# SilverlightningY/dmmt-jpeg-encoder

Hardware: AMD Instinct MI355X
Metric: Mpixel/s encoded (4K PPM, q=90) (higher is better)
Workload: dtype f32; 1 GPU; 3840x2160 synthetic RGB u8, 4:4:4, IJG quality 90, 1 frame(s) per step per GPU, pixels in HBM -> JPEG files in HBM, inputs rotating over 12 distinct slots (285 MiB: streamed from HBM); width=3840, height=2160, subsampling=P444, quality=90, parallelism=independent frames x1, lanes=4, input_slots=12

## Files before the change

dmmt-jpeg-encoder_amd/csrc/entropy.hip:

```cpp
#include <hip/hip_runtime.h>
#include <stdint.h>

#include "device_common.hpp"
#include "jpeg_common.hpp"
#include "kernels.hpp"
#include "slot_copy.hpp"

namespace dmmt {

#ifdef DMMT_PHASE_TRACE
static __device__ unsigned long long g_trace[64];
#endif

static_assert(kChunkBlocks == 256 || kChunkBlocks == 512, "one thread per block, one workgroup per chunk");
constexpr int kEmitThreads = kChunkBlocks;
constexpr int kEmitWaves = kEmitThreads / 64;
#ifndef DMMT_EMIT_OCC
#define DMMT_EMIT_OCC 7
#endif
constexpr int kEmitOcc = kChunkBlocks == 256 ? DMMT_EMIT_OCC : 3;

constexpr int kEmitWords = 4 * kChunkBlocks;
constexpr int kStuffPass = 4096;
#ifndef DMMT_EMIT_BRANCHFREE
#define DMMT_EMIT_BRANCHFREE 1
#endif
#ifndef DMMT_TAIL_DMA
#define DMMT_TAIL_DMA 1
#endif
#ifndef DMMT_TAIL_NSEG1
#define DMMT_TAIL_NSEG1 1
#endif
#ifndef DMMT_EMIT_PRIO_ALWAYS
#define DMMT_EMIT_PRIO_ALWAYS 0
#endif
#ifndef DMMT_EMIT_PRIO
#define DMMT_EMIT_PRIO 1
#endif

struct ChunkSpan {
    long long el0;
    int nb;
    int seg;
    bool seg_first, seg_last;
};

__device__ __forceinline__ ChunkSpan chunk_span(const Geom& g, int c) {
    ChunkSpan r;
    r.seg = min(c / g.cps, g.nseg - 1);
    const int j = c - r.seg * g.cps;
    const long long sb = (long long)r.seg * g.seg_blocks;
    const long long se = min(sb + g.seg_blocks, g.bpf);
    r.el0 = sb + (long long)j * kChunkBlocks;
    r.nb = (int)min((long long)kChunkBlocks, se - r.el0);
    r.seg_first = j == 0;
    r.seg_last = r.el0 + r.nb == se;
    return r;
}

__device__ __forceinline__ bool joined_tail(const Geom& g, int c) {
    return c == g.nch - 1 && g.more_after && g.restart_interval == 0;
}

__device__ __forceinline__ int mod_small(int x, int d, uint32_t inv16) {
    return x - (int)__umul24((uint32_t)d, __umul24((uint32_t)x, inv16) >> 16);
}

struct BlockCoef {
    uint32_t w[32];
};

__device__ __forceinline__ void load_block(const int16_t* __restrict__ p, BlockCoef& b) {
    const uint4* q = reinterpret_cast<const uint4*>(p);
#pragma unroll
    for (int i = 0; i < 8; ++i) {
        const uint4 v = q[i];
        b.w[4 * i] = v.x;
        b.w[4 * i + 1] = v.y;
        b.w[4 * i + 2] = v.z;
        b.w[4 * i + 3] = v.w;
    }
}

__device__ __forceinline__ int coef_at(const BlockCoef& b, int k) {
    return (k & 1) ? ((int)b.w[k >> 1] >> 16) : (int)(int16_t)(b.w[k >> 1] & 0xFFFFu);
}

__device__ __forceinline__ void zigzag_in_registers(BlockCoef& b) {
    uint32_t z[32];
#pragma unroll
    for (int j = 0; j < 32; ++j) {
        const int i0 = coef_pos(2 * j), i1 = coef_pos(2 * j + 1);
        const uint32_t lo = (b.w[i0 >> 1] >> (16 * (i0 & 1))) & 0xFFFFu;
        const uint32_t hi = (b.w[i1 >> 1] >> (16 * (i1 & 1))) & 0xFFFFu;
        z[j] = lo | (hi << 16);
    }
#pragma unroll
    for (int j = 0; j < 32; ++j) b.w[j] = z[j];
}

template <typename Sink>
__device__ __forceinline__ void walk_block(const BlockCoef& b, int dcd, const uint2* __restrict__ dctab,
                                           const uint2* __restrict__ actab, Sink& sink, int kmax = 63) {
    {
        const int cat = category_of(dcd);
        const uint2 e = dctab[cat];
        sink(e.x | extra_bits(dcd, cat), (int)e.y);
    }
    const uint2 z = actab[0xF0];
    uint32_t m_run = 0xF0u, m_low = 0xFFFFu, m_zrl = 255u;
    asm volatile("" : "+s"(m_run), "+s"(m_low), "+s"(m_zrl));
    int l16 = 16;
#pragma unroll
    for (int k0 = 0; k0 < 64; k0 += 4) {
        if (k0 != 0 && k0 > kmax) break;
#pragma unroll
        for (int k = k0 ? k0 : 1; k < k0 + 4; ++k) {
            const uint32_t w = b.w[k >> 1];
            if ((k & 1) ? w > m_low : (w << 16) != 0u) {
                const int v = coef_at(b, k);
                const int r16 = 16 * k - l16;
                if (k >= 17 && __builtin_amdgcn_ballot_w64((uint32_t)r16 > m_zrl) != 0) {
                    int r = r16 >> 8;
                    asm volatile("" : "+v"(r));
#pragma unroll 1
                    for (; r > 0; --r) sink(z.x, (int)z.y);
                }
                const int cat = category_fast(v);
                const uint2 e = actab[(r16 & (int)m_run) | cat];
                sink(e.x | extra_bits(v, cat), (int)e.y);
                l16 = 16 * k + 16;
            }
        }
    }
    if (l16 < 16 * 64 || kmax < 63) {
        const uint2 e = actab[0];
        sink(e.x, (int)e.y);
    }
}

struct CountSink {
    uint32_t n = 0;
    __device__ __forceinline__ void operator()(uint32_t, int len) { n += (uint32_t)len; }
};

struct WindowSink {
    uint32_t* img;
    int lo, n;
    unsigned long long acc;
    int nacc;
    int w;
    bool first;
    __device__ __forceinline__ void put(uint32_t word, bool shared) {
        const int i = w - lo;
        if ((unsigned)i < (unsigned)n) {
            if (shared)
                atomicOr(&img[i], word);
            else
                img[i] = word;
        }
    }
    __device__ __forceinline__ void operator()(uint32_t val, int len) {
        acc = (acc << len) | val;
        nacc += len;
        if (nacc >= 32) {
            nacc -= 32;
            put((uint32_t)(acc >> nacc), first);
            first = false;
            ++w;
        }
    }
    __device__ __forceinline__ void finish() {
        if (nacc > 0) put((uint32_t)(acc << (32 - nacc)), true);
    }
};


struct SlotSink {
    uint32_t* slot;
    unsigned long long acc;
    int nacc;
    int wi;
#if DMMT_EMIT_BRANCHFREE
    __device__ __forceinline__ void operator()(uint32_t val, int len) {
        acc = (acc << len) | val;
        nacc += len;
        const int full = nacc >> 5;
        nacc &= 31;
        slot[min(wi, kSlotWords - 1) * kEmitThreads] = (uint32_t)(acc >> nacc);
        wi += full;
    }
#else
    __device__ __forceinline__ void operator()(uint32_t val, int len) {
        acc = (acc << len) | val;
        nacc += len;
        if (nacc >= 32) {
            nacc -= 32;
            slot[min(wi, kSlotWords - 1) * kEmitThreads] = (uint32_t)(acc >> nacc);
            ++wi;
        }
    }
#endif
    __device__ __forceinline__ uint32_t finish() {
        if (nacc > 0 && wi < kSlotWords) slot[wi * kEmitThreads] = (uint32_t)(acc << (32 - nacc));
        return (uint32_t)wi * 32u + (uint32_t)nacc;
    }
};


__device__ __forceinline__ uint32_t bits16_at(uint32_t a, uint32_t b, int p) {
    const unsigned long long x = ((unsigned long long)a << 32) | b;
    return (uint32_t)(x >> (48 - (p & 31))) & 0xFFFFu;
}

struct NoMark {
    template <typename I>
    __device__ void operator()(I) const {}
};
template <typename Mark = NoMark>
__device__ __forceinline__ void fused_offsets(const uint32_t* __restrict__ cbits, const uint32_t* __restrict__ cff,
                              const unsigned long long* __restrict__ cff8, uint8_t* sFF8,
                              const uint32_t* __restrict__ cedge, const Geom& g, unsigned long long* __restrict__ bit0,
                              unsigned long long* __restrict__ outo, unsigned long long* __restrict__ total,
                              unsigned long long* sWaveV, int* sWaveF, Mark mark = Mark());
static_assert(kArriveWords == kArriveFrameWords, "the host sizes the counters");

__global__ __launch_bounds__(kEmitThreads, kEmitOcc) void k_emit(const int16_t* coef, const int16_t* __restrict__ dcdiff,
                                              const uint8_t* __restrict__ lastnz,
                                              const uint32_t* __restrict__ code_tab, Geom g,
                                              uint32_t* __restrict__ stage, uint32_t* __restrict__ chunk_bits,
                                              uint32_t* __restrict__ chunk_ff, uint32_t* __restrict__ chunk_edge,
                                              uint32_t* __restrict__ ac_hist, uint32_t* __restrict__ dc_hist,
                                              int fuse, uint32_t* __restrict__ arrive,
                                              unsigned long long* __restrict__ chunk_bit0,
                                              unsigned long long* __restrict__ chunk_out,
                                              unsigned long long* __restrict__ total_out,
                                              unsigned long long* __restrict__ chunk_ff8, int prio) {
    __shared__ uint2 sTab[2 * 256 + 2 * 16];
    __shared__ uint32_t sW[kEmitWords + 2];
    __shared__ __attribute__((aligned(16))) uint32_t sSlot[kSlotWords * kEmitThreads];
    __shared__ uint32_t sWave[kEmitWaves];
    __shared__ uint32_t sFF[8];
    __shared__ uint32_t sEdge[3];
    __shared__ uint32_t sBin[65];
    __shared__ unsigned long long sOffV[kEmitWaves + 1];
    __shared__ int sOffF[kEmitWaves];
    __shared__ uint32_t sLast;
    using OrderT = std::conditional_t<(kEmitThreads > 256), uint16_t, uint8_t>;
    uint32_t* const sBits = sW;
    OrderT* const sOrder = reinterpret_cast<OrderT*>(sW + kEmitThreads);
    uint8_t* const sKey = reinterpret_cast<uint8_t*>(sW + kEmitThreads + kEmitThreads * (int)sizeof(OrderT) / 4);
    DMMT_TRACE_START;
    const int tid = threadIdx.x, lane = lane_id(), wave = tid >> 6;
    const int frame = blockIdx.y;
    const unsigned chunk = blockIdx.x;
    const ChunkSpan span = chunk_span(g, (int)chunk);
    const long long el0 = span.el0;
    const int nb = span.nb;
    const long long e = (long long)frame * g.bpf + el0 + tid;
    const size_t cid = (size_t)frame * g.nch + chunk;
    const int r0 = (int)((uint32_t)el0 % (uint32_t)g.bpm);
    const uint32_t inv16 = (65536u + (uint32_t)g.bpm - 1u) / (uint32_t)g.bpm;
    const bool valid = tid < nb;
    const uint32_t* ct = code_tab + (size_t)frame * 1024;
    const int tt = tid & 255;
    const uint32_t tac0 = ct[256 + tt], tac1 = ct[768 + tt];
    const uint32_t tdc = ct[((tt & 31) < 16 ? 0 : 512 - 16) + (tt & 31)];
    const uint32_t lz = lastnz[valid ? e : (long long)frame * g.bpf + el0];
    if (tid < 256) {
        const int c = tid & 15;
        sTab[tid] = make_uint2((tac0 & 0xFFFFu) << c, (tac0 >> 16) + c);
        sTab[256 + tid] = make_uint2((tac1 & 0xFFFFu) << c, (tac1 >> 16) + c);
    }
    if (tid < 32) sTab[512 + tid] = make_uint2((tdc & 0xFFFFu) << (tid & 15), (tdc >> 16) + (tid & 15));
    if (chunk == 0) {
        for (int i = tid; i < kHistReps * 512; i += kEmitThreads) ac_hist[(size_t)frame * kHistReps * 512 + i] = 0u;
        for (int i = tid; i < kHistReps * 32; i += kEmitThreads) dc_hist[(size_t)frame * kHistReps * 32 + i] = 0u;
    }
    if (tid < 8) sFF[tid] = 0u;
    if (tid < 3) sEdge[tid] = 0u;
    if (tid < 65) sBin[tid] = 0u;
    const int key = valid ? (int)lz : 64;
    __syncthreads();
    const uint32_t rank = atomicAdd(&sBin[key], 1u);
    __syncthreads();
    if (tid < 64) {
        const uint32_t c = sBin[tid];
        const uint32_t inc = wave_incl_scan_full_u32(c);
        sBin[tid] = inc - c;
    }
    __syncthreads();
    const int mine = valid ? (int)(sBin[key] + rank) : tid;
    if (valid) {
        sOrder[mine] = (OrderT)tid;
        sKey[mine] = (uint8_t)key;
    }
    __syncthreads();
    DMMT_TRACE(0);
    uint32_t wbits = 0;
    bool slot_over = false;
    {
#if DMMT_EMIT_PRIO
        if (prio) {
            if (wave == 3) __builtin_amdgcn_s_setprio(3);
            else if (wave == 2) __builtin_amdgcn_s_setprio(2);
            else if (wave == 1) __builtin_amdgcn_s_setprio(1);
        }
#endif
        if (valid) {
            const int p = sOrder[tid];
            const long long ep = (long long)frame * g.bpf + el0 + p;
            BlockCoef b;
            load_block(coef + ep * 64, b);
            zigzag_in_registers(b);
            const int dp = dcdiff[ep];
            DMMT_TRACE(4);
            const int kp = mod_small(r0 + p, g.bpm, inv16);
            const bool lum = kp < g.n_luma;
            const int kmax = __builtin_amdgcn_readfirstlane((int)sKey[min(64 * wave + 63, nb - 1)]);
            SlotSink ss{sSlot + tid, 0ull, 0, 0};
            walk_block(b, dp, sTab + 512 + (lum ? 0 : 16), sTab + (lum ? 0 : 256), ss, kmax);
            wbits = ss.finish();
            slot_over = wbits > (uint32_t)kSlotWords * 32u;
            sBits[p] = wbits;
            DMMT_TRACE(5);
        }
    }
#if DMMT_EMIT_PRIO
    if (prio) __builtin_amdgcn_s_setprio(0);
#endif
    const bool over = __syncthreads_or(slot_over) != 0;
    const uint32_t bits = valid ? sBits[tid] : 0u;
    const int k = valid ? mod_small(r0 + tid, g.bpm, inv16) : 0;
    const bool lum_t = k < g.n_luma;
    const uint32_t incl = wave_incl_scan_full_u32(bits);
    if (lane == 63) sWave[wave] = incl;
    __syncthreads();
    uint32_t start = incl - bits;
    uint32_t total = 0;
#pragma unroll
    for (int q = 0; q < kEmitWaves; ++q) {
        start += q < wave ? sWave[q] : 0u;
        total += sWave[q];
    }
    DMMT_TRACE(1);

    uint32_t* slot = stage + cid * (size_t)kChunkWordsCap;
    const int nw = (int)((total + 31) >> 5);
    const int we1 = total >= 16 ? (int)((total - 16) >> 5) : 0;
    uint32_t ff[8] = {0, 0, 0, 0, 0, 0, 0, 0};
    for (int w0 = 0; w0 < nw; w0 += kEmitWords) {
        const int wn = min(kEmitWords, nw - w0);
        if (!over) {
            SlotWords sw;
            read_slot<kEmitThreads>(sSlot, mine, bits, sw);
            if (tid == 0 && w0 + wn >= nw) sW[wn] = 0u;
            copy_owned(sw, start, bits, sW, w0, wn);
            __syncthreads();
            copy_head(sw, start, bits, sW, w0, wn);
        } else {
            for (int i = tid; i <= wn; i += kEmitThreads) sW[i] = 0u;
            __syncthreads();
        }
        if (over && bits && start < (uint32_t)(w0 + wn + 1) * 32u && start + bits > (uint32_t)w0 * 32u) {
            {
                BlockCoef b;
                load_block(coef + e * 64, b);
                zigzag_in_registers(b);
                WindowSink ws{sW, w0, wn + 1, 0ull, (int)(start & 31), (int)(start >> 5), true};
                walk_block(b, dcdiff[e], sTab + 512 + (lum_t ? 0 : 16), sTab + (lum_t ? 0 : 256), ws);
                ws.finish();
            }
        }
        __syncthreads();
        for (int i = tid; i < wn; i += kEmitThreads) {
            const uint32_t a = sW[i], c = sW[i + 1];
            slot[w0 + i] = a;
            const int wi = w0 + i;
            if (wi == 0) sEdge[0] = a;
            if (wi == we1) {
                sEdge[1] = a;
                sEdge[2] = c;
            }
            const unsigned long long x = ((unsigned long long)a << 32) | c;
            unsigned long long z = x & (x << 1);
            z &= z << 2;
            z &= z << 4;
            const uint32_t m = (uint32_t)(z >> 32);
            if (m) {
#pragma unroll
                for (int r = 0; r < 8; ++r) ff[r] += __popc(m & (0x80808080u >> r));
            }
        }
        __syncthreads();
    }
    DMMT_TRACE(2);
#pragma unroll
    for (int r = 0; r < 4; ++r) {
        const uint32_t v = wave_sum_full_u32(ff[2 * r] | (ff[2 * r + 1] << 16));
        if (lane == 0 && v) {
            atomicAdd(&sFF[2 * r], v & 0xFFFFu);
            atomicAdd(&sFF[2 * r + 1], v >> 16);
        }
    }
    __syncthreads();
    if (tid == 0) {
        const uint32_t first16 = sEdge[0] >> 16;
        uint32_t last16;
        if (total >= 16)
            last16 = bits16_at(sEdge[1], sEdge[2], (int)(total - 16));
        else
            last16 = total ? sEdge[0] >> (32 - total) : 0u;
        unsigned long long f8 = 0;
#pragma unroll
        for (int r = 0; r < 8; ++r) {
            __hip_atomic_store(chunk_ff + cid * 8 + r, sFF[r], __ATOMIC_RELAXED, __HIP_MEMORY_SCOPE_AGENT);
            f8 |= (unsigned long long)min(sFF[r], 255u) << (8 * r);
        }
        __hip_atomic_store(chunk_ff8 + cid, f8, __ATOMIC_RELAXED, __HIP_MEMORY_SCOPE_AGENT);
        __hip_atomic_store(chunk_bits + cid, total, __ATOMIC_RELAXED, __HIP_MEMORY_SCOPE_AGENT);
        __hip_atomic_store(chunk_edge + cid, (first16 << 16) | last16, __ATOMIC_RELAXED, __HIP_MEMORY_SCOPE_AGENT);
    }
    if (fuse) {
        if (tid == 0) sLast = arrive_last(arrive + (size_t)frame * kArriveWords, chunk, (unsigned)g.nch);
        __syncthreads();
        DMMT_TRACE(6);
        if (sLast) {
            arrive_acquire();
            const size_t fb = (size_t)frame * g.nch;
#ifdef DMMT_PHASE_TRACE
            auto mark = [&](auto i) { DMMT_TRACE(decltype(i)::value); };
#else
            NoMark mark;
#endif
            fused_offsets(chunk_bits + fb, chunk_ff + fb * 8, chunk_ff8 + fb, reinterpret_cast<uint8_t*>(sSlot),
                          chunk_edge + fb, g, chunk_bit0 + fb, chunk_out + fb, total_out + frame, sOffV, sOffF, mark);
        }
    }
    DMMT_TRACE(3);
    DMMT_TRACE_FLUSH(0, 0);
}

__device__ __forceinline__ uint32_t boundary_byte(int m1, uint32_t last16, bool has_next, uint32_t n_next,
                                                  uint32_t first16_next) {
    uint32_t v = last16 & ((1u << m1) - 1u);
    int m2 = 8 - m1;
    if (has_next) {
        const int t = (int)min((uint32_t)m2, n_next);
        v = (v << t) | (t ? first16_next >> (16 - t) : 0u);
        m2 -= t;
    }
    return ((v << m2) | ((1u << m2) - 1u)) & 0xFFu;
}

__device__ __forceinline__ unsigned long long chunk_out_bytes(const uint32_t* __restrict__ cff,
                                                              const uint32_t* __restrict__ cbits,
                                                              const uint32_t* __restrict__ cedge, const Geom& g,
                                                              int c, unsigned long long b0) {
    const ChunkSpan sp = chunk_span(g, c);
    const uint32_t n = cbits[c];
    const unsigned long long e = b0 + n;
    unsigned long long out = ((e + 7) >> 3) - ((b0 + 7) >> 3);
    out += cff[(size_t)c * 8 + ((8 - (b0 & 7)) & 7)];
    if ((e & 7) && (e & ~7ull) >= b0) {
        const bool jt = joined_tail(g, c);
        const bool has_next = !sp.seg_last || jt;
        const uint32_t nn = jt ? (uint32_t)g.next_bits : (has_next ? cbits[c + 1] : 0u);
        const uint32_t fn = jt ? g.next16 : (has_next ? cedge[c + 1] >> 16 : 0u);
        const uint32_t byte = boundary_byte((int)(e & 7), cedge[c] & 0xFFFFu, has_next, nn, fn);
        out += byte == 0xFFu ? 1u : 0u;
    }
    if (sp.seg_last && (c != g.nch - 1 || (g.more_after && g.restart_interval > 0))) out += 2;
    return out;
}

template <int NW>
__device__ __forceinline__ unsigned long long block_scan_nw(unsigned long long v, unsigned long long* sWave,
                                                            unsigned long long* tot) {
    const int lane = lane_id(), wave = threadIdx.x >> 6;
    const unsigned long long incl = wave_incl_scan_full_u64(v);
    if (lane == 63) sWave[wave] = incl;
    __syncthreads();
    unsigned long long pre = incl - v, all = 0;
    for (int q = 0; q < NW; ++q) {
        if (q < wave) pre += sWave[q];
        all += sWave[q];
    }
    __syncthreads();
    *tot = all;
    return pre;
}

__device__ __forceinline__ void seg_combine(bool& f, unsigned long long& v, bool f2, unsigned long long v2) {
    v = f2 ? v2 : v + v2;
    f = f || f2;
}

template <int NW>
__device__ __forceinline__ unsigned long long block_segscan_nw(bool f, unsigned long long v,
                                                               unsigned long long* sWaveV, int* sWaveF,
                                                               bool* flag_out = nullptr) {
    const int lane = lane_id(), wave = threadIdx.x >> 6;
    bool fi = f;
    unsigned long long vi = v;
    auto step = [&](unsigned long long pv, int pf) {
        bool ff = pf != 0;
        seg_combine(ff, pv, fi, vi);
        fi = ff;
        vi = pv;
    };
    step(dpp_u64<0x111, 0xF, 0xF, true>(vi), __builtin_amdgcn_update_dpp(0, (int)fi, 0x111, 0xF, 0xF, true));
    step(dpp_u64<0x112, 0xF, 0xF, true>(vi), __builtin_amdgcn_update_dpp(0, (int)fi, 0x112, 0xF, 0xF, true));
    step(dpp_u64<0x114, 0xF, 0xF, true>(vi), __builtin_amdgcn_update_dpp(0, (int)fi, 0x114, 0xF, 0xF, true));
    step(dpp_u64<0x118, 0xF, 0xF, true>(vi), __builtin_amdgcn_update_dpp(0, (int)fi, 0x118, 0xF, 0xF, true));
    step(dpp_u64<0x142, 0xA, 0xF, false>(vi), __builtin_amdgcn_update_dpp(0, (int)fi, 0x142, 0xA, 0xF, false));
    step(dpp_u64<0x143, 0xC, 0xF, false>(vi), __builtin_amdgcn_update_dpp(0, (int)fi, 0x143, 0xC, 0xF, false));
    if (lane == 63) {
        sWaveV[wave] = vi;
        sWaveF[wave] = fi;
    }
    const unsigned long long ve = dpp_u64<0x138, 0xF, 0xF, true>(vi);
    const int fe = __builtin_amdgcn_update_dpp(0, (int)fi, 0x138, 0xF, 0xF, true);
    __syncthreads();
    bool cf = false;
    unsigned long long cv = 0;
    for (int q = 0; q < wave; ++q) seg_combine(cf, cv, sWaveF[q] != 0, sWaveV[q]);
    bool rf = cf;
    unsigned long long rv = cv;
    seg_combine(rf, rv, fe != 0, ve);
    __syncthreads();
    if (flag_out) *flag_out = rf;
    return rv;
}

__device__ __forceinline__ unsigned long long block_scan_1024(unsigned long long v, unsigned long long* sWave,
                                                              unsigned long long* tot) {
    return block_scan_nw<16>(v, sWave, tot);
}
__device__ __forceinline__ unsigned long long block_segscan_1024(bool f, unsigned long long v,
                                                                 unsigned long long* sWaveV, int* sWaveF) {
    return block_segscan_nw<16>(f, v, sWaveV, sWaveF);
}

static_assert(kFusedRoundChunks % kEmitThreads == 0, "whole chunks per thread of the fused offsets");
static_assert(kFusedRoundChunks % (2 * kEmitThreads) == 0 && kFusedRoundChunks * 8 <= kSlotWords * kEmitThreads * 4,
              "a round's packed 0xFF counts: whole 16-byte pieces per thread, inside k_emit's slot area");
static_assert((unsigned long long)kFusedOffsetsMaxChunks * kChunkBlocks * kMaxBlockBits < (1ull << 32),
              "a fused frame's bit offsets fit 32 bits");
template <typename Mark>
__device__ __forceinline__ void fused_offsets(const uint32_t* __restrict__ cbits, const uint32_t* __restrict__ cff,
                              const unsigned long long* __restrict__ cff8, uint8_t* sFF8,
                              const uint32_t* __restrict__ cedge, const Geom& g, unsigned long long* __restrict__ bit0,
                              unsigned long long* __restrict__ outo, unsigned long long* __restrict__ total,
                              unsigned long long* sWaveV, int* sWaveF, Mark mark) {
    constexpr int KP = kFusedRoundChunks / kEmitThreads, NT = kEmitThreads;
    const int tid = threadIdx.x;
    const int nch = g.nch;
    uint32_t carry_run = 0, carry_out = 0;
    for (int r0 = 0; r0 < nch; r0 += kFusedRoundChunks) {
        const int rn = min(kFusedRoundChunks, nch - r0);
        const int per = (rn + NT - 1) / NT;
        const int c0 = r0 + min(tid * per, rn), c1 = r0 + min(tid * per + per, rn);
#if DMMT_TAIL_DMA
        {
            const int npairs = (rn + 1) >> 1;
#pragma unroll
            for (int i = 0; i < kFusedRoundChunks / 2 / NT; ++i) {
                const int pc = min(i * NT + tid, npairs - 1);
                __builtin_amdgcn_global_load_lds((const void*)(cff8 + r0 + 2 * pc),
                                                 (void*)(sFF8 + 16 * (i * NT + (tid & ~63))), 16, 0, 16);
            }
        }
#endif
        uint32_t nbits[KP], edge[KP];
#pragma unroll
        for (int i = 0; i < KP; ++i) {
            const int c = min(c0 + i, nch - 1);
            nbits[i] = ld_agent(cbits + c);
            edge[i] = ld_agent(cedge + c);
        }
        const int cl = min(c1, nch - 1);
        const uint32_t nlast = ld_agent(cbits + cl), elast = ld_agent(cedge + cl);
        uint32_t firstm = 0, seglm = 0;
#pragma unroll
        for (int i = 0; i < KP; ++i) nbits[i] = c0 + i < c1 ? nbits[i] : 0u;
        if (DMMT_TAIL_NSEG1 && g.nseg == 1) {
            firstm = c0 == 0 && c0 < c1 ? 1u : 0u;
            seglm = c1 == nch && c0 < c1 ? 1u << (c1 - 1 - c0) : 0u;
        } else {
#pragma unroll
            for (int i = 0; i < KP; ++i) {
                const int c = c0 + i;
                if (c < c1) {
                    const ChunkSpan sp = chunk_span(g, c);
                    firstm |= (uint32_t)sp.seg_first << i;
                    seglm |= (uint32_t)sp.seg_last << i;
                }
            }
        }
        bool f = false;
        unsigned long long v = 0;
#pragma unroll
        for (int i = 0; i < KP; ++i)
            if (c0 + i < c1) seg_combine(f, v, (firstm >> i) & 1u, nbits[i] + (c0 + i == 0 ? (uint32_t)g.bit_phase : 0u));
        bool fx;
        const uint32_t ex = (uint32_t)block_segscan_nw<kEmitWaves>(f, v, sWaveV, sWaveF, &fx);
        mark(std::integral_constant<int, 7>{});
        uint32_t run = fx ? ex : carry_run + ex;
        uint32_t b0[KP];
#pragma unroll
        for (int i = 0; i < KP; ++i) {
            b0[i] = 0;
            if (c0 + i < c1) {
                if ((firstm >> i) & 1u) run = c0 + i == 0 ? (uint32_t)g.bit_phase : 0u;
                b0[i] = run;
                run += nbits[i];
            }
        }
        if (c0 < c1 && c1 == r0 + rn) sWaveV[kEmitWaves] = run;
        uint32_t ob[KP];
#if DMMT_TAIL_DMA
#pragma unroll
        for (int i = 0; i < KP; ++i) {
            const int cc = min(c0 + i, nch - 1);
            const uint32_t slot = (8u - (b0[i] & 7u)) & 7u;
            ob[i] = sFF8[8 * (cc - r0) + slot];
            if (ob[i] == 255u) ob[i] = ld_agent(cff + (size_t)cc * 8 + slot);
        }
#else
#pragma unroll
        for (int i = 0; i < KP; ++i)
            ob[i] = ld_agent(cff + (size_t)min(c0 + i, nch - 1) * 8 + ((8 - (b0[i] & 7)) & 7));
#endif
        uint32_t mine = 0;
#pragma unroll
        for (int i = 0; i < KP; ++i) {
            const int c = c0 + i;
            if (c >= c1) {
                ob[i] = 0;
                continue;
            }
            const uint32_t e = b0[i] + nbits[i];
            uint32_t o = ((e + 7) >> 3) - ((b0[i] + 7) >> 3) + ob[i];
            if ((e & 7) && (e & ~7u) >= b0[i]) {
                const bool segl = (seglm >> i) & 1u;
                const bool jt = segl && joined_tail(g, c);
                const bool hasn = !segl || jt;
                const uint32_t nn = jt ? (uint32_t)g.next_bits : i + 1 < KP && c + 1 < c1 ? nbits[min(i + 1, KP - 1)] : nlast;
                const uint32_t en = jt ? g.next16 << 16 : i + 1 < KP && c + 1 < c1 ? edge[min(i + 1, KP - 1)] : elast;
                const uint32_t byte = boundary_byte((int)(e & 7), edge[i] & 0xFFFFu, hasn, nn, en >> 16);
                o += byte == 0xFFu ? 1u : 0u;
            }
            if (((seglm >> i) & 1u) && (c != nch - 1 || (g.more_after && g.restart_interval > 0))) o += 2;
            ob[i] = o;
            mine += o;
        }
        mark(std::integral_constant<int, 8>{});
        unsigned long long tot = 0;
        uint32_t orun = carry_out + (uint32_t)block_scan_nw<kEmitWaves>(mine, sWaveV, &tot);
        mark(std::integral_constant<int, 9>{});
#pragma unroll
        for (int i = 0; i < KP; ++i) {
            const int c = c0 + i;
            if (c >= c1) continue;
            bit0[c] = b0[i];
            outo[c] = orun;
            orun += ob[i];
        }
        carry_out += (uint32_t)tot;
        carry_run = (uint32_t)sWaveV[kEmitWaves];
        __syncthreads();
        mark(std::integral_constant<int, 10>{});
    }
    if (tid == 0) *total = carry_out;
}

__global__ __launch_bounds__(1024) void k_offsets(const uint32_t* __restrict__ chunk_bits,
                                                  const uint32_t* __restrict__ chunk_ff,
                                                  const uint32_t* __restrict__ chunk_edge, Geom g,
                                                  unsigned long long* __restrict__ chunk_bit0,
                                                  unsigned long long* __restrict__ chunk_out,
                                                  unsigned long long* __restrict__ total_out) {
    __shared__ unsigned long long sWave[16];
    __shared__ int sWaveF[16];
    const int tid = threadIdx.x;
    const int frame = blockIdx.x;
    const int nch = g.nch;
    const uint32_t* cbits = chunk_bits + (size_t)frame * nch;
    const uint32_t* cff = chunk_ff + (size_t)frame * nch * 8;
    const uint32_t* cedge = chunk_edge + (size_t)frame * nch;
    unsigned long long* bit0 = chunk_bit0 + (size_t)frame * nch;
    unsigned long long* outo = chunk_out + (size_t)frame * nch;
    const int per = (nch + 1023) / 1024;
    const int c0 = min(tid * per, nch), c1 = min(c0 + per, nch);

    constexpr int KP = 2;
    if (per <= KP) {
        uint32_t nbits[KP], ffr[KP][8], edge[KP], nnext[KP], enext[KP];
        bool first[KP], segl[KP], hasn[KP];
#pragma unroll
        for (int i = 0; i < KP; ++i) {
            const int c = c0 + i;
            nbits[i] = edge[i] = nnext[i] = enext[i] = 0u;
            first[i] = segl[i] = hasn[i] = false;
#pragma unroll
            for (int r = 0; r < 8; ++r) ffr[i][r] = 0u;
            if (c < c1) {
                const ChunkSpan sp = chunk_span(g, c);
                first[i] = sp.seg_first;
                segl[i] = sp.seg_last;
                hasn[i] = !sp.seg_last;
                nbits[i] = cbits[c];
// ... 194 lines not shown
        if (lane == 63) sWave[wave] = incl;
        __syncthreads();
        uint32_t pre = incl - cnt;
        for (int q = 0; q < wave; ++q) pre += sWave[q];
        const uint32_t ffs = sWave[0] + sWave[1] + sWave[2] + sWave[3];
        if (nvalid) {
            const uint32_t dst = delta + (uint32_t)tid * 16u + pre;
            uint32_t a = dst;
#pragma unroll
            for (int i = 0; i < 4; ++i) {
                const uint32_t w = x[i], f = ffm[i];
                sOut[a + 4 * i] = (uint8_t)(w >> 24);
                sOut[a + (uint32_t)__popc(f & 0x80000000u) + 4 * i + 1] = (uint8_t)(w >> 16);
                sOut[a + (uint32_t)__popc(f & 0x80800000u) + 4 * i + 2] = (uint8_t)(w >> 8);
                sOut[a + (uint32_t)__popc(f & 0x80808000u) + 4 * i + 3] = (uint8_t)w;
                a += (uint32_t)__popc(f);
            }
            if (cnt) {
                uint32_t m = 0;
#pragma unroll
                for (int i = 0; i < 4; ++i)
                    m |= ((((ffm[i] >> 7) * 0x08040201u) >> 24) & 0xFu) << (4 * i);
                uint32_t z = dst + 1;
                while (m) {
                    sOut[z + (uint32_t)__builtin_ctz(m)] = 0x00;
                    ++z;
                    m &= m - 1u;
                }
            }
        }
        __syncthreads();
        const unsigned long long in_pass = nbytes - pos < (unsigned long long)kStuffPass ? nbytes - pos : kStuffPass;
        const uint32_t len = (uint32_t)in_pass + ffs;
        const uint32_t send = delta + len;
        uint8_t* const oa = o - delta;
        for (uint32_t sb = 16u * (uint32_t)tid; sb + 16u <= send; sb += 16u * 256u) {
            if (sb >= delta) *reinterpret_cast<uint4*>(oa + sb) = *reinterpret_cast<const uint4*>(sOut + sb);
        }
        if (tid < 32) {
            const uint32_t sbt = send & ~15u;
            const uint32_t i = tid < 16 ? (uint32_t)tid : sbt + (uint32_t)tid - 16u;
            const bool mine = tid < 16 ? i >= delta && (delta > 0u || send < 16u) : sbt > 0u;
            if (mine && i < send) oa[i] = sOut[i];
        }
        o += len;
        __syncthreads();
    }
}

bool offsets_fusable(const Geom& g) { return g.nch <= kFusedOffsetsMaxChunks; }

hipError_t launch_emit(int n_frames, const Geom& g, const Work& w, bool fuse_offsets, hipStream_t st, bool prio) {
    const int fuse = fuse_offsets && offsets_fusable(g) ? 1 : 0;
    hipLaunchKernelGGL(k_emit, dim3(g.nch, n_frames), dim3(kEmitThreads), 0, st, (const int16_t*)w.coef,
                       (const int16_t*)w.dcdiff, (const uint8_t*)w.lastnz, (const uint32_t*)w.code_tab, g, w.stage, w.chunk_bits, w.chunk_ff,
                       w.chunk_edge, w.ac_hist, w.dc_hist, fuse, w.arrive, w.chunk_bit0, w.chunk_out, w.total_out,
                       w.chunk_ff8, prio || DMMT_EMIT_PRIO_ALWAYS ? 1 : 0);
    return hipGetLastError();
}

hipError_t launch_offsets(int n_frames, const Geom& g, const Work& w, hipStream_t st) {
    hipLaunchKernelGGL(k_offsets, dim3(n_frames), dim3(1024), 0, st, (const uint32_t*)w.chunk_bits,
                       (const uint32_t*)w.chunk_ff, (const uint32_t*)w.chunk_edge, g, w.chunk_bit0, w.chunk_out,
                       w.total_out);
    return hipGetLastError();
}

hipError_t launch_stuffwrite(int n_frames, const Geom& g, const Work& w, uint8_t* out, size_t out_stride,
                             uint32_t* out_len, hipStream_t st) {
    hipLaunchKernelGGL(k_stuffwrite, dim3(g.nch, n_frames), dim3(256), 0, st, (const uint32_t*)w.stage,
                       (const uint32_t*)w.chunk_bits, (const uint32_t*)w.chunk_edge,
                       (const unsigned long long*)w.chunk_bit0, (const unsigned long long*)w.chunk_out,
                       (const unsigned long long*)w.total_out, (const uint32_t*)w.hdr_len, g, out, out_stride,
                       out_len, w.status);
    return hipGetLastError();
}

}

#ifdef DMMT_PHASE_TRACE
extern "C" int dmmt_debug_trace_entropy(unsigned long long* out64) {
    if (hipMemcpyFromSymbol(out64, HIP_SYMBOL(dmmt::g_trace), 64 * 8) != hipSuccess) return -1;
    unsigned long long z[64] = {0};
    return hipMemcpyToSymbol(HIP_SYMBOL(dmmt::g_trace), z, sizeof z) == hipSuccess ? 0 : -1;
}
#endif
```

dmmt-jpeg-encoder_amd/csrc/kernels.hip:

```cpp

#include <hip/hip_runtime.h>
#include <stdint.h>
#include <stdlib.h>

#include <type_traits>

#include "dct_quant.hpp"
#include "device_common.hpp"
#include "front_launch.hpp"
#include "jpeg_common.hpp"
#include "kernels.hpp"
#include "surface_load.hpp"
#include "wave_merge.hpp"

namespace dmmt {

#ifdef DMMT_PHASE_TRACE
static __device__ unsigned long long g_trace[64];
#endif

__constant__ uint8_t c_zigzag[64] = {0,  1,  8,  16, 9,  2,  3,  10, 17, 24, 32, 25, 18, 11, 4,  5,
                                     12, 19, 26, 33, 40, 48, 41, 34, 27, 20, 13, 6,  7,  14, 21, 28,
                                     35, 42, 49, 56, 57, 50, 43, 36, 29, 22, 15, 23, 30, 37, 44, 51,
                                     58, 59, 52, 45, 38, 31, 39, 46, 53, 60, 61, 54, 47, 55, 62, 63};
// ... 432 lines not shown
            if (blk < NYB) {
                const int by = blk / 32, bx = blk % 32;
                el = (bx / HR) * BPM + by * HR + (bx % HR);
            } else if (blk < NYB + CB) {
                el = (blk - NYB) * BPM + NLUMA;
            } else {
                el = (blk - NYB - CB) * BPM + NLUMA + 1;
            }
            const bool valid = el < nvalid;
            if (valid) {
                uint32_t pk[4];
#pragma unroll
                for (int i = 0; i < 4; ++i) pk[i] = __builtin_amdgcn_perm((uint32_t)x[2 * i + 1], (uint32_t)x[2 * i], 0x05040100u);
                *reinterpret_cast<uint4*>(cbase + (el * 64 + 8 * col)) = make_uint4(pk[0], pk[1], pk[2], pk[3]);
            }
        }
        DMMT_TRACE(2);
    }

    if (bad) raise_status(status, bad);
    DMMT_TRACE(5);
    DMMT_TRACE_FLUSH(0, 0);
}

template <int HR, int VR, typename Sample, int WPE>
__global__ __launch_bounds__(256, WPE) void k_front(const Sample* __restrict__ rgb, size_t frame_stride, Geom g,
                                               const float* __restrict__ norm_lut,
                                               const float* __restrict__ qtab,
                                               int16_t* __restrict__ coef, int* __restrict__ status) {
    front_body<HR, VR, Sample, LAY_TIGHT>(rgb, frame_stride, SurfArgs{}, g, norm_lut, qtab, coef, status);
}

template <int HR, int VR, typename Sample, int LAY, int WPE>
__global__ __launch_bounds__(256, WPE) void k_front_surf(SurfArgs sa, size_t frame_stride, Geom g,
                                                    const float* __restrict__ norm_lut,
                                                    const float* __restrict__ qtab, int16_t* __restrict__ coef,
                                                    int* __restrict__ status) {
    front_body<HR, VR, Sample, LAY>(nullptr, frame_stride, sa, g, norm_lut, qtab, coef, status);
}

struct HistCoef {
    uint32_t w[32];
};

constexpr int kTailSmallWords = 4 + 4 * 16;
__device__ __forceinline__ void tables_tail(uint8_t* lds, const uint32_t* ac_hist, const uint32_t* dc_hist, int frame,
                                            const Geom& g, uint32_t* __restrict__ code_tab, uint8_t* __restrict__ out,
                                            size_t out_stride, uint32_t* __restrict__ hdr_len,
                                            const uint8_t* __restrict__ qtab_u8, int bits_per_channel,
                                            int* __restrict__ status, int* sCnt, int* sBits);
constexpr int kHistCopies = 4, kHistCopyWords = 545;
constexpr int kTailLdsBytes = 7072;

template <bool CHECK, bool FUSE>
__global__ __launch_bounds__(256) __attribute__((amdgpu_waves_per_eu(8, 8))) void k_hist(const int16_t* __restrict__ coef, int16_t* __restrict__ dcdiff,
                                              uint8_t* __restrict__ lastnz, Geom g,
                                              uint32_t* __restrict__ ac_hist ,
                                              uint32_t* __restrict__ dc_hist ,
                                              int* __restrict__ status, uint32_t* __restrict__ arrive,
                                              uint32_t* __restrict__ code_tab, uint8_t* __restrict__ out,
                                              size_t out_stride, uint32_t* __restrict__ hdr_len,
                                              const uint8_t* __restrict__ qtab_u8, int bits_per_channel) {
    constexpr int NC = kHistCopies, HS = kHistCopyWords;
    constexpr int kWords = FUSE && kTailLdsBytes / 4 > NC * HS ? kTailLdsBytes / 4 : NC * HS;
    __shared__ __attribute__((aligned(16))) uint32_t sH[kWords];
    __shared__ int sSmall[FUSE ? kTailSmallWords : 1];
    __shared__ uint32_t sLastWg;
    const int tid = threadIdx.x;
    const int frame = blockIdx.y;
    for (int i = tid; i < NC * HS; i += 256) sH[i] = 0;
    __syncthreads();
    uint32_t* const H = sH + HS * (tid & 3);
    const long long base = (long long)frame * g.bpf;
    const int lane = lane_id();
    int bad = 0;
    const uint32_t bpf = (uint32_t)g.bpf, bpm = (uint32_t)g.bpm, ri = (uint32_t)max(g.restart_interval, 1);
    const uint32_t stride = gridDim.x * 256u, sm = stride / bpm, sk = stride - sm * bpm;
    uint32_t el = blockIdx.x * 256u + (uint32_t)tid;
    uint32_t m = el / bpm, k = el - m * bpm, mr = m % ri;
    const uint32_t smr = sm % ri;
    for (; el < bpf; el += stride) {
        const long long e = base + el;
        const uint4* q = reinterpret_cast<const uint4*>(coef + e * 64);
        uint32_t cw[32];
#pragma unroll
        for (int i = 0; i < 8; ++i) {
            const uint4 v = q[i];
            cw[4 * i] = v.x, cw[4 * i + 1] = v.y, cw[4 * i + 2] = v.z, cw[4 * i + 3] = v.w;
        }
        const int t = k < (uint32_t)g.n_luma ? 0 : 1;
        const bool restart = g.restart_interval > 0 && mr == 0;
        int back = 0;
        if (k > 0 && k < (uint32_t)g.n_luma)
            back = 1;
        else if (m > 0 && !restart)
            back = (k == 0) ? (int)bpm - g.n_luma + 1 : (int)bpm;
        const int cur = (int)(int16_t)(cw[0] & 0xFFFFu);
        const int nb = __shfl_up(cur, (unsigned)back, 64);
        int pv = 0;
        if (back) pv = lane >= back ? nb : (int)coef[(e - back) * 64];
        HistCoef b;
#pragma unroll
        for (int j = 0; j < 32; ++j) {
            const int i0 = coef_pos(2 * j), i1 = coef_pos(2 * j + 1);
            const uint32_t lo = (cw[i0 >> 1] >> (16 * (i0 & 1))) & 0xFFFFu;
            const uint32_t hi = (cw[i1 >> 1] >> (16 * (i1 & 1))) & 0xFFFFu;
            b.w[j] = lo | (hi << 16);
        }
        uint32_t* h = H + 256 * t;
        int l16 = 16;
        uint32_t zrl = 0;
#pragma unroll
        for (int kk = 1; kk < 64; ++kk) {
            const int v = (kk & 1) ? ((int)b.w[kk >> 1] >> 16) : (int)(int16_t)(b.w[kk >> 1] & 0xFFFFu);
            if (v != 0) {
                if (CHECK && v == -32768) bad |= 4;
                const int r16 = 16 * kk - l16;
                zrl += (uint32_t)(r16 >> 8);
                atomicAdd(&h[(r16 & 0xF0) | category_fast(v)], 1u);
                l16 = 16 * kk + 16;
            }
        }
        if (zrl) atomicAdd(&h[0xF0], zrl);
        if (l16 < 16 * 64) atomicAdd(&h[0], 1u);
        lastnz[e] = (uint8_t)((l16 >> 4) - 1);
        {
            const int16_t d = (int16_t)(cur - pv);
            bad |= d == -32768 ? 4 : 0;
            dcdiff[e] = d;
            atomicAdd(&H[512 + 16 * t + category_of(d)], 1u);
        }
        m += sm, k += sk, mr += smr;
        if (k >= bpm) k -= bpm, ++m, ++mr;
        if (mr >= ri) mr -= ri;
    }
    if (bad) raise_status(status, bad);
    __syncthreads();
    const size_t rep = (size_t)frame * kHistReps + blockIdx.x % kHistReps;
    for (int i = tid; i < 544; i += 256) {
        uint32_t v = 0;
#pragma unroll
        for (int c = 0; c < NC; ++c) v += sH[HS * c + i];
        if (!v) continue;
        if (i < 512)
            atomicAdd(&ac_hist[rep * 512 + i], v);
        else
            atomicAdd(&dc_hist[rep * 32 + (i - 512)], v);
    }
    if (FUSE) {
#if !DMMT_ARRIVE_FORMAL
        asm volatile("s_waitcnt vmcnt(0)" ::: "memory");
#endif
        __syncthreads();
        if (tid == 0) sLastWg = arrive_last(arrive + (size_t)frame * kArriveWords, blockIdx.x, gridDim.x);
        __syncthreads();
        if (sLastWg) {
            arrive_acquire();
            tables_tail(reinterpret_cast<uint8_t*>(sH), ac_hist, dc_hist, frame, g, code_tab, out, out_stride, hdr_len,
                        qtab_u8, bits_per_channel, status, sSmall, sSmall + 4);
        }
    }
}


#define PM_LEVELS 15

__device__ __forceinline__ void put_be16(uint8_t* p, int v) {
    p[0] = (uint8_t)(v >> 8);
    p[1] = (uint8_t)v;
}

__device__ void write_table_header(uint8_t* o, int tab, int t0, int step, int n, const int nt[4],
                                   const uint8_t* symrank, const int* bits16, const Geom& g,
                                   const uint8_t* __restrict__ qtab_u8, int bits_per_channel, uint32_t* hdr_len,
                                   int dq = -1) {
    if (!g.stripe_first) {
        if (tab == 0 && t0 == 0) *hdr_len = 0;
        return;
    }
    const int pos_dht0 = 2 + 18 + 69 + 69 + 19;
    const int off_lac = pos_dht0;
    const int off_ldc = off_lac + 21 + nt[1];
    const int off_cac = off_ldc + 21 + nt[0];
    const int off_cdc = off_cac + 21 + nt[3];
    const int dht = tab == 0 ? off_ldc : tab == 1 ? off_lac : tab == 2 ? off_cdc : off_cac;
    for (int s = t0; s < n; s += step) o[dht + 21 + s] = symrank[n - 1 - s];
    for (int s = t0; s < 16; s += step) o[dht + 5 + s] = (uint8_t)bits16[s];
// ... 786 lines not shown
```

Before: 194,100 Mpixel/s.

## Cut emit kernel LDS and registers, skip zigzag via column-major walk, raise occupancy

The emit kernel's window buffer now aliases the slot area in LDS, with a separate small sort area, which reduces shared-memory use. The kernel is templated on occupancy: 8 waves for the single-frame case and 7 for batched non-priority launches. Thread id, mine index and lane are recomputed after the walk (mine is packed into the upper bits of sBits) instead of being held live, and ff counters are packed into 4 registers, all to lower register pressure. The walker reads coefficients in zigzag order through coef_pos, so the register zigzag permutation is skipped. The ZRL table load moves inside its rare branch. A disabled newest-first hist traversal option is also added.

```diff
diff --git a/dmmt-jpeg-encoder_amd/csrc/entropy.hip b/dmmt-jpeg-encoder_amd/csrc/entropy.hip
--- a/dmmt-jpeg-encoder_amd/csrc/entropy.hip
+++ b/dmmt-jpeg-encoder_amd/csrc/entropy.hip
@@ -16,9 +16,13 @@
 constexpr int kEmitThreads = kChunkBlocks;
 constexpr int kEmitWaves = kEmitThreads / 64;
 #ifndef DMMT_EMIT_OCC
-#define DMMT_EMIT_OCC 7
+#define DMMT_EMIT_OCC 8
 #endif
 constexpr int kEmitOcc = kChunkBlocks == 256 ? DMMT_EMIT_OCC : 3;
+#ifndef DMMT_EMIT_OCC_BATCH
+#define DMMT_EMIT_OCC_BATCH 7
+#endif
+constexpr int kEmitOccBatch = kChunkBlocks == 256 ? DMMT_EMIT_OCC_BATCH : 3;
 
 constexpr int kEmitWords = 4 * kChunkBlocks;
 constexpr int kStuffPass = 4096;
@@ -30,6 +34,9 @@
 #endif
 #ifndef DMMT_TAIL_NSEG1
 #define DMMT_TAIL_NSEG1 1
+#endif
+#ifndef DMMT_WALK_COLUMN_MAJOR
+#define DMMT_WALK_COLUMN_MAJOR 1
 #endif
 #ifndef DMMT_EMIT_PRIO_ALWAYS
 #define DMMT_EMIT_PRIO_ALWAYS 0
@@ -87,6 +94,9 @@
 }
 
 __device__ __forceinline__ void zigzag_in_registers(BlockCoef& b) {
+#if DMMT_WALK_COLUMN_MAJOR
+    return;
+#endif
     uint32_t z[32];
 #pragma unroll
     for (int j = 0; j < 32; ++j) {
@@ -107,7 +117,6 @@
         const uint2 e = dctab[cat];
         sink(e.x | extra_bits(dcd, cat), (int)e.y);
     }
-    const uint2 z = actab[0xF0];
     uint32_t m_run = 0xF0u, m_low = 0xFFFFu, m_zrl = 255u;
     asm volatile("" : "+s"(m_run), "+s"(m_low), "+s"(m_zrl));
     int l16 = 16;
@@ -116,13 +125,15 @@
         if (k0 != 0 && k0 > kmax) break;
 #pragma unroll
         for (int k = k0 ? k0 : 1; k < k0 + 4; ++k) {
-            const uint32_t w = b.w[k >> 1];
-            if ((k & 1) ? w > m_low : (w << 16) != 0u) {
-                const int v = coef_at(b, k);
+            const int kc =DMMT_WALK_COLUMN_MAJOR ? coef_pos(k) : k;
+            const uint32_t w = b.w[kc >> 1];
+            if ((kc & 1) ? w > m_low : (w << 16) != 0u) {
+                const int v = coef_at(b, kc);
                 const int r16 = 16 * k - l16;
                 if (k >= 17 && __builtin_amdgcn_ballot_w64((uint32_t)r16 > m_zrl) != 0) {
                     int r = r16 >> 8;
                     asm volatile("" : "+v"(r));
+                    const uint2 z = actab[0xF0];
 #pragma unroll 1
                     for (; r > 0; --r) sink(z.x, (int)z.y);
                 }
@@ -222,10 +233,17 @@
                               const unsigned long long* __restrict__ cff8, uint8_t* sFF8,
                               const uint32_t* __restrict__ cedge, const Geom& g, unsigned long long* __restrict__ bit0,
                               unsigned long long* __restrict__ outo, unsigned long long* __restrict__ total,
-                              unsigned long long* sWaveV, int* sWaveF, Mark mark = Mark());
+                              unsigned long long* sWaveV, int* sWaveF, int tid, Mark mark = Mark());
 static_assert(kArriveWords == kArriveFrameWords, "the host sizes the counters");
 
-__global__ __launch_bounds__(kEmitThreads, kEmitOcc) void k_emit(const int16_t* coef, const int16_t* __restrict__ dcdiff,
+__device__ __forceinline__ int tid_again(int wave) {
+    uint32_t zero = 0u;
+    asm volatile("" : "+s"(zero));
+    return (wave << 6) | (int)__builtin_amdgcn_mbcnt_hi(~0u, __builtin_amdgcn_mbcnt_lo(~0u, zero));
+}
+
+template <int OCC>
+__global__ __launch_bounds__(kEmitThreads, OCC) void k_emit(const int16_t* coef, const int16_t* __restrict__ dcdiff,
                                               const uint8_t* __restrict__ lastnz,
                                               const uint32_t* __restrict__ code_tab, Geom g,
                                               uint32_t* __restrict__ stage, uint32_t* __restrict__ chunk_bits,
@@ -237,8 +255,10 @@
                                               unsigned long long* __restrict__ total_out,
                                               unsigned long long* __restrict__ chunk_ff8, int prio) {
     __shared__ uint2 sTab[2 * 256 + 2 * 16];
-    __shared__ uint32_t sW[kEmitWords + 2];
     __shared__ __attribute__((aligned(16))) uint32_t sSlot[kSlotWords * kEmitThreads];
+    static_assert(kEmitWords + 2 <= kSlotWords * kEmitThreads, "the window image lies inside the slot area");
+    uint32_t* const sW = sSlot;
+    __shared__ uint32_t sSort[kEmitThreads + kEmitThreads * (int)sizeof(std::conditional_t<(kEmitThreads > 256), uint16_t, uint8_t>) / 4 + kEmitThreads / 4];
     __shared__ uint32_t sWave[kEmitWaves];
     __shared__ uint32_t sFF[8];
     __shared__ uint32_t sEdge[3];
@@ -247,26 +267,26 @@
     __shared__ int sOffF[kEmitWaves];
     __shared__ uint32_t sLast;
     using OrderT = std::conditional_t<(kEmitThreads > 256), uint16_t, uint8_t>;
-    uint32_t* const sBits = sW;
-    OrderT* const sOrder = reinterpret_cast<OrderT*>(sW + kEmitThreads);
-    uint8_t* const sKey = reinterpret_cast<uint8_t*>(sW + kEmitThreads + kEmitThreads * (int)sizeof(OrderT) / 4);
+    uint32_t* const sBits = sSort;
+    OrderT* const sOrder = reinterpret_cast<OrderT*>(sSort + kEmitThreads);
+    uint8_t* const sKey = reinterpret_cast<uint8_t*>(sSort + kEmitThreads + kEmitThreads * (int)sizeof(OrderT) / 4);
     DMMT_TRACE_START;
-    const int tid = threadIdx.x, lane = lane_id(), wave = tid >> 6;
+    int tid = threadIdx.x;
+    const int wave = __builtin_amdgcn_readfirstlane(tid >> 6);
     const int frame = blockIdx.y;
     const unsigned chunk = blockIdx.x;
     const ChunkSpan span = chunk_span(g, (int)chunk);
     const long long el0 = span.el0;
     const int nb = span.nb;
-    const long long e = (long long)frame * g.bpf + el0 + tid;
     const size_t cid = (size_t)frame * g.nch + chunk;
     const int r0 = (int)((uint32_t)el0 % (uint32_t)g.bpm);
     const uint32_t inv16 = (65536u + (uint32_t)g.bpm - 1u) / (uint32_t)g.bpm;
-    const bool valid = tid < nb;
+    bool valid = tid < nb;
     const uint32_t* ct = code_tab + (size_t)frame * 1024;
     const int tt = tid & 255;
     const uint32_t tac0 = ct[256 + tt], tac1 = ct[768 + tt];
     const uint32_t tdc = ct[((tt & 31) < 16 ? 0 : 512 - 16) + (tt & 31)];
-    const uint32_t lz = lastnz[valid ? e : (long long)frame * g.bpf + el0];
+    const uint32_t lz = lastnz[(long long)frame * g.bpf + el0 + (valid ? tid : 0)];
     if (tid < 256) {
         const int c = tid & 15;
         sTab[tid] = make_uint2((tac0 & 0xFFFFu) << c, (tac0 >> 16) + c);
@@ -290,8 +310,8 @@
         sBin[tid] = inc - c;
     }
     __syncthreads();
-    const int mine = valid ? (int)(sBin[key] + rank) : tid;
     if (valid) {
+        const int mine = (int)(sBin[key] + rank);
         sOrder[mine] = (OrderT)tid;
         sKey[mine] = (uint8_t)key;
     }
@@ -322,7 +342,7 @@
             walk_block(b, dp, sTab + 512 + (lum ? 0 : 16), sTab + (lum ? 0 : 256), ss, kmax);
             wbits = ss.finish();
             slot_over = wbits > (uint32_t)kSlotWords * 32u;
-            sBits[p] = wbits;
+            sBits[p] = wbits | ((uint32_t)tid << 16);
             DMMT_TRACE(5);
         }
     }
@@ -330,9 +350,13 @@
     if (prio) __builtin_amdgcn_s_setprio(0);
 #endif
     const bool over = __syncthreads_or(slot_over) != 0;
-    const uint32_t bits = valid ? sBits[tid] : 0u;
-    const int k = valid ? mod_small(r0 + tid, g.bpm, inv16) : 0;
-    const bool lum_t = k < g.n_luma;
+    tid = tid_again(wave);
+    const int lane = tid & 63;
+    valid = tid < nb;
+    static_assert(kMaxBlockBits < (1 << 16), "a block's bit count and its walker's column share a word");
+    const uint32_t bw = valid ? sBits[tid] : (uint32_t)tid << 16;
+    const uint32_t bits = bw & 0xFFFFu;
+    const int mine = (int)(bw >> 16);
     const uint32_t incl = wave_incl_scan_full_u32(bits);
     if (lane == 63) sWave[wave] = incl;
     __syncthreads();
@@ -348,31 +372,8 @@
     uint32_t* slot = stage + cid * (size_t)kChunkWordsCap;
     const int nw = (int)((total + 31) >> 5);
     const int we1 = total >= 16 ? (int)((total - 16) >> 5) : 0;
-    uint32_t ff[8] = {0, 0, 0, 0, 0, 0, 0, 0};
-    for (int w0 = 0; w0 < nw; w0 += kEmitWords) {
-        const int wn = min(kEmitWords, nw - w0);
-        if (!over) {
-            SlotWords sw;
-            read_slot<kEmitThreads>(sSlot, mine, bits, sw);
-            if (tid == 0 && w0 + wn >= nw) sW[wn] = 0u;
-            copy_owned(sw, start, bits, sW, w0, wn);
-            __syncthreads();
-            copy_head(sw, start, bits, sW, w0, wn);
-        } else {
-            for (int i = tid; i <= wn; i += kEmitThreads) sW[i] = 0u;
-            __syncthreads();
-        }
-        if (over && bits && start < (uint32_t)(w0 + wn + 1) * 32u && start + bits > (uint32_t)w0 * 32u) {
-            {
-                BlockCoef b;
-                load_block(coef + e * 64, b);
-                zigzag_in_registers(b);
-                WindowSink ws{sW, w0, wn + 1, 0ull, (int)(start & 31), (int)(start >> 5), true};
-                walk_block(b, dcdiff[e], sTab + 512 + (lum_t ? 0 : 16), sTab + (lum_t ? 0 : 256), ws);
-                ws.finish();
-            }
-        }
-        __syncthreads();
+    uint32_t ff[4] = {0, 0, 0, 0};
+    auto window_out = [&](int tid, int w0, int wn) {
         for (int i = tid; i < wn; i += kEmitThreads) {
             const uint32_t a = sW[i], c = sW[i + 1];
             slot[w0 + i] = a;
@@ -389,15 +390,55 @@
             const uint32_t m = (uint32_t)(z >> 32);
             if (m) {
 #pragma unroll
-                for (int r = 0; r < 8; ++r) ff[r] += __popc(m & (0x80808080u >> r));
-            }
-        }
+                for (int r = 0; r < 4; ++r)
+                    ff[r] += __popc(m & (0x80808080u >> (2 * r))) | (__popc(m & (0x80808080u >> (2 * r + 1))) << 16);
+            }
+        }
+    };
+    if (!over) {
+        SlotWords sw;
+        read_slot<kEmitThreads>(sSlot, mine, bits, sw);
         __syncthreads();
+        for (int w0 = 0; w0 < nw; w0 += kEmitWords) {
+            const int wn = min(kEmitWords, nw - w0);
+            uint32_t st = start;
+            asm volatile("" : "+v"(st));
+            if (tid == 0 && w0 + wn >= nw) sW[wn] = 0u;
+            copy_owned(sw, st, bits, sW, w0, wn);
+            __syncthreads();
+            copy_head(sw, st, bits, sW, w0, wn);
+            __syncthreads();
+            window_out(tid, w0, wn);
+            __syncthreads();
+        }
+    } else {
+        for (int w0 = 0; w0 < nw; w0 += kEmitWords) {
+            const int wn = min(kEmitWords, nw - w0);
+            uint32_t st = start;
+            asm volatile("" : "+v"(st));
+            for (int i = tid; i <= wn; i += kEmitThreads) sW[i] = 0u;
+            __syncthreads();
+            if (bits && st < (uint32_t)(w0 + wn + 1) * 32u && st + bits > (uint32_t)w0 * 32u) {
+                const int te = tid_again(wave);
+                const long long e = (long long)frame * g.bpf + el0 + te;
+                const bool lum_t = mod_small(r0 + te, g.bpm, inv16) < g.n_luma;
+                BlockCoef b;
+                load_block(coef + e * 64, b);
+                zigzag_in_registers(b);
+                WindowSink ws{sW, w0, wn + 1, 0ull, (int)(st & 31), (int)(st >> 5), true};
+                walk_block(b, dcdiff[e], sTab + 512 + (lum_t ? 0 : 16), sTab + (lum_t ? 0 : 256), ws);
+                ws.finish();
+            }
+            tid = tid_again(wave);
+            __syncthreads();
+            window_out(tid, w0, wn);
+            __syncthreads();
+        }
     }
     DMMT_TRACE(2);
 #pragma unroll
     for (int r = 0; r < 4; ++r) {
-        const uint32_t v = wave_sum_full_u32(ff[2 * r] | (ff[2 * r + 1] << 16));
+        const uint32_t v = wave_sum_full_u32(ff[r]);
         if (lane == 0 && v) {
             atomicAdd(&sFF[2 * r], v & 0xFFFFu);
             atomicAdd(&sFF[2 * r + 1], v >> 16);
@@ -434,7 +475,7 @@
             NoMark mark;
 #endif
             fused_offsets(chunk_bits + fb, chunk_ff + fb * 8, chunk_ff8 + fb, reinterpret_cast<uint8_t*>(sSlot),
-                          chunk_edge + fb, g, chunk_bit0 + fb, chunk_out + fb, total_out + frame, sOffV, sOffF, mark);
+                          chunk_edge + fb, g, chunk_bit0 + fb, chunk_out + fb, total_out + frame, sOffV, sOffF, tid, mark);
         }
     }
     DMMT_TRACE(3);
@@ -476,8 +517,8 @@
 
 template <int NW>
 __device__ __forceinline__ unsigned long long block_scan_nw(unsigned long long v, unsigned long long* sWave,
-                                                            unsigned long long* tot) {
-    const int lane = lane_id(), wave = threadIdx.x >> 6;
+                                                            unsigned long long* tot, int tid = threadIdx.x) {
+    const int lane = tid & 63, wave = __builtin_amdgcn_readfirstlane(tid >> 6);
     const unsigned long long incl = wave_incl_scan_full_u64(v);
     if (lane == 63) sWave[wave] = incl;
     __syncthreads();
@@ -499,8 +540,8 @@
 template <int NW>
 __device__ __forceinline__ unsigned long long block_segscan_nw(bool f, unsigned long long v,
                                                                unsigned long long* sWaveV, int* sWaveF,
-                                                               bool* flag_out = nullptr) {
-    const int lane = lane_id(), wave = threadIdx.x >> 6;
+                                                               bool* flag_out = nullptr, int tid = threadIdx.x) {
+    const int lane = tid & 63, wave = __builtin_amdgcn_readfirstlane(tid >> 6);
     bool fi = f;
     unsigned long long vi = v;
     auto step = [&](unsigned long long pv, int pf) {
@@ -552,9 +593,8 @@
                               const unsigned long long* __restrict__ cff8, uint8_t* sFF8,
                               const uint32_t* __restrict__ cedge, const Geom& g, unsigned long long* __restrict__ bit0,
                               unsigned long long* __restrict__ outo, unsigned long long* __restrict__ total,
-                              unsigned long long* sWaveV, int* sWaveF, Mark mark) {
+                              unsigned long long* sWaveV, int* sWaveF, int tid, Mark mark) {
     constexpr int KP = kFusedRoundChunks / kEmitThreads, NT = kEmitThreads;
-    const int tid = threadIdx.x;
     const int nch = g.nch;
     uint32_t carry_run = 0, carry_out = 0;
     for (int r0 = 0; r0 < nch; r0 += kFusedRoundChunks) {
@@ -604,7 +644,7 @@
         for (int i = 0; i < KP; ++i)
             if (c0 + i < c1) seg_combine(f, v, (firstm >> i) & 1u, nbits[i] + (c0 + i == 0 ? (uint32_t)g.bit_phase : 0u));
         bool fx;
-        const uint32_t ex = (uint32_t)block_segscan_nw<kEmitWaves>(f, v, sWaveV, sWaveF, &fx);
+        const uint32_t ex = (uint32_t)block_segscan_nw<kEmitWaves>(f, v, sWaveV, sWaveF, &fx, tid);
         mark(std::integral_constant<int, 7>{});
         uint32_t run = fx ? ex : carry_run + ex;
         uint32_t b0[KP];
@@ -657,7 +697,7 @@
         }
         mark(std::integral_constant<int, 8>{});
         unsigned long long tot = 0;
-        uint32_t orun = carry_out + (uint32_t)block_scan_nw<kEmitWaves>(mine, sWaveV, &tot);
+        uint32_t orun = carry_out + (uint32_t)block_scan_nw<kEmitWaves>(mine, sWaveV, &tot, tid);
         mark(std::integral_constant<int, 9>{});
 #pragma unroll
         for (int i = 0; i < KP; ++i) {
@@ -958,7 +998,8 @@
 
 hipError_t launch_emit(int n_frames, const Geom& g, const Work& w, bool fuse_offsets, hipStream_t st, bool prio) {
     const int fuse = fuse_offsets && offsets_fusable(g) ? 1 : 0;
-    hipLaunchKernelGGL(k_emit, dim3(g.nch, n_frames), dim3(kEmitThreads), 0, st, (const int16_t*)w.coef,
+    const auto kern = !prio && n_frames > 1 ? k_emit<kEmitOccBatch> : k_emit<kEmitOcc>;
+    hipLaunchKernelGGL(kern, dim3(g.nch, n_frames), dim3(kEmitThreads), 0, st, (const int16_t*)w.coef,
                        (const int16_t*)w.dcdiff, (const uint8_t*)w.lastnz, (const uint32_t*)w.code_tab, g, w.stage, w.chunk_bits, w.chunk_ff,
                        w.chunk_edge, w.ac_hist, w.dc_hist, fuse, w.arrive, w.chunk_bit0, w.chunk_out, w.total_out,
                        w.chunk_ff8, prio || DMMT_EMIT_PRIO_ALWAYS ? 1 : 0);
diff --git a/dmmt-jpeg-encoder_amd/csrc/kernels.hip b/dmmt-jpeg-encoder_amd/csrc/kernels.hip
--- a/dmmt-jpeg-encoder_amd/csrc/kernels.hip
+++ b/dmmt-jpeg-encoder_amd/csrc/kernels.hip
@@ -508,6 +508,9 @@
 constexpr int kHistCopies = 4, kHistCopyWords = 545;
 constexpr int kTailLdsBytes = 7072;
 
+#ifndef DMMT_HIST_NEWEST_FIRST
+#define DMMT_HIST_NEWEST_FIRST 0
+#endif
 template <bool CHECK, bool FUSE>
 __global__ __launch_bounds__(256) __attribute__((amdgpu_waves_per_eu(8, 8))) void k_hist(const int16_t* __restrict__ coef, int16_t* __restrict__ dcdiff,
                                               uint8_t* __restrict__ lastnz, Geom g,
@@ -533,9 +536,21 @@
     const uint32_t bpf = (uint32_t)g.bpf, bpm = (uint32_t)g.bpm, ri = (uint32_t)max(g.restart_interval, 1);
     const uint32_t stride = gridDim.x * 256u, sm = stride / bpm, sk = stride - sm * bpm;
     uint32_t el = blockIdx.x * 256u + (uint32_t)tid;
+#if DMMT_HIST_NEWEST_FIRST
+    const uint32_t passes = (bpf + stride - 1u) / stride;
+    el += (passes - 1u) * stride;
+    const uint32_t el1 = el < bpf ? el : el - stride;
+    uint32_t m = el1 / bpm, k = el1 - m * bpm, mr = m % ri;
+#else
     uint32_t m = el / bpm, k = el - m * bpm, mr = m % ri;
+#endif
     const uint32_t smr = sm % ri;
+#if DMMT_HIST_NEWEST_FIRST
+    for (uint32_t left = passes; left > 0; --left, el -= stride) {
+        if (el >= bpf) continue;
+#else
     for (; el < bpf; el += stride) {
+#endif
         const long long e = base + el;
         const uint4* q = reinterpret_cast<const uint4*>(coef + e * 64);
         uint32_t cw[32];
@@ -586,9 +601,15 @@
             dcdiff[e] = d;
             atomicAdd(&H[512 + 16 * t + category_of(d)], 1u);
         }
+#if DMMT_HIST_NEWEST_FIRST
+        m -= sm, k -= sk, mr -= smr;
+        if (k >= bpm) k += bpm, --m, --mr;
+        if (mr >= ri) mr += ri;
+#else
         m += sm, k += sk, mr += smr;
         if (k >= bpm) k -= bpm, ++m, ++mr;
         if (mr >= ri) mr -= ri;
+#endif
     }
     if (bad) raise_status(status, bad);
     __syncthreads();
```

New measurement: 200,400 Mpixel/s (median of 6 runs). +3.2%, better.
